# barronalex/Tacotron

Measured on AMD Instinct MI355X. Metric: mel-frames/sec (train step, batch=32 r=2), higher is better.
Workload: dtype f32

## Files before the change

include/taco_hip.h:

```cpp
#ifndef TACO_HIP_H
#define TACO_HIP_H

#include <stddef.h>
#include <stdint.h>

#ifdef __cplusplus
extern "C" {
#endif
#pragma GCC visibility push(default)

#define TACO_VERSION 120

#define TACO_OK 0
#define TACO_EINVAL (-1)
#define TACO_ELAUNCH (-2)
#define TACO_ENOTFOUND (-3)

#define TACO_ACT_NONE 0
#define TACO_ACT_RELU 1
#define TACO_ACT_SIGMOID 2
#define TACO_ACT_TANH 3

typedef struct TacoShape {
  int32_t B;
// ... 66 lines not shown
                                  int taps, int T, int pad_l, void* stream);
int taco_debug_bn_maxpool_fwd(const float* x, const float* gamma, const float* beta, float* y, int B, int T, int C, void* stream);
int taco_debug_bn_maxpool_bwd(const float* x, const float* gamma, const float* beta, const float* dy, float* dx, float* dgamma,
                              float* dbeta, int B, int T, int C, void* stream);
int taco_debug_bank_gather(const float* dbank, int lda, const float* const* WT, const float* residual, int ldr, float* dx_out, int ldc,
                           float* slabs, int64_t slab_floats, int M, int T, int F, int K, int N, int pad_l, int S, void* stream);
int taco_debug_conv_gemm_batch_atomic(const float* dbank, int lda, const float* const* WT, const float* residual, int ldr, float* dx_out,
                                      int ldc, int M, int T, int F, int K, int N, void* stream);
int taco_debug_conv_gemm_rowbias(const float* A, int lda, const float* W, int ldw, const float* rowb, int bias_stride, float* C, int ldc,
                                 int M, int T, int N, int K, void* stream);
int taco_debug_gemm_tn_group(int n, const float* const* A, const int* lda, const float* const* Y, const int* ldy, float* const* W,
                             const int* ldw, float* const* dbias, const int* M, const int* N, const int* K, const int* taps,
                             const int* T, const int* pad_l, void* stream);
int taco_debug_gemm_tn_strided(const float* A, int lda, int64_t strideA, const float* Y, int ldy, int64_t strideY, float* W, int ldw,
                               int64_t strideW, int M, int N, int K, int T, int pad_l, int batch, void* stream);

int taco_debug_embedding(const float* table, const int32_t* ids, float* out, int rows, int V, int width, void* stream);
int taco_debug_embedding_bwd(const float* dout, const int32_t* ids, float* dtable, int rows, int V, int width, void* stream);
int taco_debug_highway_combine(const float* th, const float* x, float* y, int M, void* stream);
int taco_debug_highway_combine_bwd(const float* th, const float* x, const float* dy, float* dth, float* dx, int M, void* stream);
int taco_debug_act_bwd(const float* y, const float* dy, const uint8_t* keep, float* dz, int64_t n, int act, void* stream);
int taco_debug_affine_act_bwd(const float* pre, const float* gamma, const float* dy, float* dz, float* dgamma, float* dbeta, int M,
                              int N, int act, void* stream);
int taco_debug_colsum_batched(const float* x, int ld, float* out, int B, int T, int N, void* stream);
int taco_debug_mask_rows(const float* x, const int32_t* len, float* y, int B, int T, int C, void* stream);
int taco_debug_center_rows(const float* x, const int32_t* len, float* out, int B, int T, int C, void* stream);
int taco_debug_mask_pos(float* g, int ldg, const float* y, int ldy, int rows, int cols, float scale, void* stream);
int taco_debug_zero_tail_rows(float* x0, int C0, float* x1, int C1, const int32_t* len, int B, int Td, void* stream);
int taco_debug_add(const float* a, const float* b, float* y, int64_t n, void* stream);
int taco_debug_l1_loss(const float* a0, const float* b0, float* grad0, int ldg0, int M0, int N0, const float* a1, const float* b1,
// ... 195 lines not shown
```

tacotron_amd/csrc/bf16x3.h:

```cpp
#pragma once
#include "common.h"

namespace {

typedef unsigned u32x4 __attribute__((ext_vector_type(4)));
typedef __bf16 bf16x8 __attribute__((ext_vector_type(8)));
struct Pl3 {
  u32x4 h, m, l;
};
__device__ __forceinline__ void split2(float x0, float x1, unsigned& h, unsigned& m, unsigned& l) {
  const unsigned u0 = __float_as_uint(x0), u1 = __float_as_uint(x1);
  h = __builtin_amdgcn_perm(u1, u0, 0x07060302u);
  const float r0 = x0 - __uint_as_float(u0 & 0xffff0000u), r1 = x1 - __uint_as_float(u1 & 0xffff0000u);
  const unsigned v0 = __float_as_uint(r0), v1 = __float_as_uint(r1);
  m = __builtin_amdgcn_perm(v1, v0, 0x07060302u);
  const float s0 = r0 - __uint_as_float(v0 & 0xffff0000u), s1 = r1 - __uint_as_float(v1 & 0xffff0000u);
  l = __builtin_amdgcn_perm(__float_as_uint(s1), __float_as_uint(s0), 0x07060302u);
}
__device__ __forceinline__ Pl3 split8(float f0, float f1, float f2, float f3, float f4, float f5, float f6, float f7) {
  unsigned h[4], m[4], l[4];
  split2(f0, f1, h[0], m[0], l[0]);
  split2(f2, f3, h[1], m[1], l[1]);
  split2(f4, f5, h[2], m[2], l[2]);
  split2(f6, f7, h[3], m[3], l[3]);
// ... 2 lines not shown
  p.m = u32x4{m[0], m[1], m[2], m[3]};
  p.l = u32x4{l[0], l[1], l[2], l[3]};
  return p;
}
__device__ __forceinline__ f32x16 mfma_bf(const u32x4& a, const u32x4& b, const f32x16& c) {
  return __builtin_amdgcn_mfma_f32_32x32x16_bf16(__builtin_bit_cast(bf16x8, a), __builtin_bit_cast(bf16x8, b), c, 0, 0, 0);
}
__device__ __forceinline__ void mfma6_2(f32x16& hi, f32x16& lo, const Pl3& a, const Pl3& b) {
  lo = mfma_bf(a.l, b.h, lo);
  hi = mfma_bf(a.h, b.h, hi);
  lo = mfma_bf(a.h, b.l, lo);
  lo = mfma_bf(a.m, b.m, lo);
  lo = mfma_bf(a.m, b.h, lo);
  lo = mfma_bf(a.h, b.m, lo);
}
__device__ __forceinline__ Pl3 zero_pl3() {
  Pl3 p;
  p.h = u32x4{0, 0, 0, 0}; p.m = p.h; p.l = p.h;
  return p;
}


inline bool env_bf16x() { return sw_on<SW_GEMM2_BF16X>(); }

inline int bf16x_max_chain() { return sw_int<SW_BF16X_MAX_CHAIN>(); }

}
```

tacotron_amd/csrc/gemm.hip:

```cpp
#include <algorithm>

#include "bf16x3.h"
#include "common.h"
#include "kernels.h"

namespace {

constexpr int BK = 16;

__device__ __forceinline__ float4 sel4(bool ok, const float4 t) {
  return make_float4(ok ? t.x : 0.f, ok ? t.y : 0.f, ok ? t.z : 0.f, ok ? t.w : 0.f);
}

struct RowInfo {
  int m;
  int t;
  bool ok;
};

template <int WM, int WN, bool VA, bool VB>
__global__ __launch_bounds__(256) void conv_gemm_kernel(ConvGemmBatch batch) {
  constexpr int BM = 64 * WM, BN = 64 * WN;
  constexpr int LDS_A = BM + 4, LDS_B = BN + 4;
  constexpr int A_PER = BM / 64;
// ... 881 lines not shown
  TACO_REQUIRE(bias_stride >= N, "%s: bias_stride must be >= N = %d, got %d", who, N, bias_stride);
  DoorOperands o;
  o.in(A, door_span(M, K, lda), "A");
  o.in(W, door_span(K, N, ldw), "W");
  o.in(rowb, door_span(M / T, N, bias_stride), "rowb");
  o.out(C, door_span(M, N, ldc), "C");
  TACO_TRY(o.check(who));
  ConvGemmProblem p;
  p.A = A; p.lda = lda; p.W = W; p.ldw = ldw; p.bias = rowb; p.C = C; p.ldc = ldc;
  p.M = M; p.N = N; p.K = K; p.taps = 1; p.pad_l = 0; p.act = TACO_ACT_NONE;
  p.T = T;
  p.bias_stride = bias_stride;
  return launch_conv_gemm(p, as_stream(stream));
}

extern "C" int taco_debug_gemm_tn_group(int n, const float* const* A, const int* lda, const float* const* Y, const int* ldy,
                                        float* const* W, const int* ldw, float* const* dbias, const int* M, const int* N, const int* K,
                                        const int* taps, const int* T, const int* pad_l, void* stream) {
  const char* who = "taco_debug_gemm_tn_group";
  TACO_REQUIRE(n >= 1 && n <= kMaxTnBatch, "%s: n must be in [1, %d], got %d", who, kMaxTnBatch, n);
  TACO_REQUIRE(A && lda && Y && ldy && W && ldw && M && N && K && taps && T && pad_l, "%s: a table is null", who);
  DoorOperands o;
  for (int i = 0; i < n; ++i) {
    TACO_REQUIRE(M[i] > 0 && M[i] <= kDoorMaxRows, "%s: M[%d] must be in [1, 2^22], got %d", who, i, M[i]);
    TACO_REQUIRE(T[i] > 0 && M[i] % T[i] == 0, "%s: T[%d] must be positive and divide M[%d] = %d, got %d", who, i, i, M[i], T[i]);
    TACO_REQUIRE(N[i] > 0 && N[i] <= kDoorMaxCols, "%s: N[%d] must be in [1, 2^14], got %d", who, i, N[i]);
    TACO_REQUIRE(K[i] > 0 && K[i] <= kDoorMaxCols, "%s: K[%d] must be in [1, 2^14], got %d", who, i, K[i]);
    TACO_REQUIRE(taps[i] >= 1 && taps[i] <= 64, "%s: taps[%d] must be in [1, 64], got %d", who, i, taps[i]);
    TACO_REQUIRE(pad_l[i] >= -64 && pad_l[i] <= 64, "%s: pad_l[%d] must be in [-64, 64], got %d", who, i, pad_l[i]);
    TACO_REQUIRE(lda[i] >= K[i], "%s: lda[%d] must be >= K = %d, got %d", who, i, K[i], lda[i]);
// ... 47 lines not shown
```

tacotron_amd/csrc/gemm2.hip:

```cpp
#include <algorithm>
#include <type_traits>

#include "bf16x3.h"
#include "common.h"
#include "kernels.h"

namespace {

__device__ __attribute__((aligned(16))) float g_zero4[4];

__device__ __forceinline__ void glds16(const float* g, float* lds_wave_base) {
  __builtin_amdgcn_global_load_lds((const __attribute__((address_space(1))) void*)g,
                                   (__attribute__((address_space(3))) void*)lds_wave_base, 16, 0, 0);
}
constexpr int kOOB = (int)0x80000000;
__device__ __forceinline__ __amdgpu_buffer_rsrc_t dma_rsrc(const float* base) {
  return __builtin_amdgcn_make_buffer_rsrc(const_cast<float*>(base), 0, 0x7fffffff, 0x00020000);
}
__device__ __forceinline__ void blds16(__amdgpu_buffer_rsrc_t rs, int voffset, int soffset, float* lds_wave_base) {
  __builtin_amdgcn_raw_ptr_buffer_load_lds(rs, (__attribute__((address_space(3))) void*)lds_wave_base, 16, voffset, soffset, 0, 0);
}
template <int N>
__device__ __forceinline__ void wait_vm() {
  asm volatile("s_waitcnt vmcnt(%0)" ::"n"(N) : "memory");
// ... 32 lines not shown
    f(std::integral_constant<int, I>{});
    static_for<I + 1, N>(f);
  }
}

constexpr int TM = 128, TN = 128;

struct Gemm2Args {
  ConvGemmBatch batch;
  int first[kMaxGemmBatch];
  int mt[kMaxGemmBatch];
  int xcd_map;
  int bk_pa[8], bk_a0[8], bk_na[8], bk_pb[8], bk_b0[8], bk_nb[8];
};

template <int BK, int NS, int BX = 0>
__global__ __launch_bounds__(256, 2) void conv_gemm2_kernel(Gemm2Args G) {
  static_assert(!BX || BK == 16, "the bf16x3 form works on 16-deep k-tiles (one v_mfma_f32_32x32x16_bf16 group per tile)");
  constexpr int SLOTS = BK / 4;
  constexpr int A_RPI = 64 / SLOTS;
  constexpr int A_INSTR = TM / A_RPI / 4;
  constexpr int B_INSTR = BX == 2 ? kWImgTileBytes / 4096 : BK / 2 / 4;
  constexpr int NLD = A_INSTR + B_INSTR;
  constexpr int A_FLOATS = TM * BK, B_FLOATS = BX == 2 ? kWImgTileBytes / 4 : BK * TN, STAGE = A_FLOATS + B_FLOATS;
  constexpr int SWZ_SH = BK == 32 ? 1 : 2;
  extern __shared__ __attribute__((aligned(16))) float smem[];

  int lin = blockIdx.x;
  int bank_pi = -1, bank_rel = 0;
  if (G.xcd_map == 2) {
    const int x = lin & 7, j = lin >> 3;
    if (j < G.bk_na[x]) { bank_pi = G.bk_pa[x]; bank_rel = G.bk_a0[x] + j; }
    else if (j < G.bk_na[x] + G.bk_nb[x]) { bank_pi = G.bk_pb[x]; bank_rel = G.bk_b0[x] + j - G.bk_na[x]; }
// ... 201 lines not shown
  auto compute_bi = [&](int stage, int fill_stage, auto fill_c) __attribute__((always_inline)) {
    constexpr bool fill = decltype(fill_c)::value;
    const uint32_t sb = lds0 + (uint32_t)stage * (STAGE * 4u);
    const uint32_t bb = sb + (uint32_t)(A_FLOATS * 4) + (uint32_t)lane * 16u;
    const f32x4 ra0 = dsr128<0>(sb + a_off[0]);
    const f32x4 ra1 = dsr128<0>(sb + a_off[NP - 1]);
    u32x4 pl[4][3];
    static_for<0, 4>([&](auto jc) {
      constexpr int j = decltype(jc)::value;
      static_for<0, 3>([&](auto pc) {
        constexpr int pp = decltype(pc)::value;
        pl[j][pp] = __builtin_bit_cast(u32x4, dsr128<(4 * pp + j) * 1024>(bb));
      });
    });
    __builtin_amdgcn_sched_barrier(0);
    acc_lo[2] = mfma_bf(pa_c.l, qb2_c.h, acc_lo[2]);
    acc_lo[3] = mfma_bf(pa_c.l, qb3_c.h, acc_lo[3]);
    acc[2] = mfma_bf(pa_c.h, qb2_c.h, acc[2]);
    acc[3] = mfma_bf(pa_c.h, qb3_c.h, acc[3]);
    acc_lo[2] = mfma_bf(pa_c.h, qb2_c.l, acc_lo[2]);
    acc_lo[3] = mfma_bf(pa_c.h, qb3_c.l, acc_lo[3]);
    if (fill) {
#pragma unroll
      for (int g = 0; g < NLD; ++g) issue_piece(g, fill_stage);
    }
    __builtin_amdgcn_sched_barrier(0);
    wait_lgkm<12>();
    __builtin_amdgcn_sched_barrier(0);
    acc_lo[2] = mfma_bf(pa_c.m, qb2_c.m, acc_lo[2]);
    acc_lo[3] = mfma_bf(pa_c.m, qb3_c.m, acc_lo[3]);
// ... 42 lines not shown
    __builtin_amdgcn_s_barrier();
    asm volatile("" ::: "memory");
    run_tile(it % NS, (it + NS - 1) % NS, std::true_type{});
    advance();
  }
  for (; it < nit; ++it) {
    wait_vm<0>();
    __builtin_amdgcn_s_barrier();
    asm volatile("" ::: "memory");
    run_tile(it % NS, 0, std::false_type{});
  }
  if constexpr (BX == 1) {
    MF6(2, pa_c, pb2_c);
    MF6(3, pa_c, pb3_c);
  }
  if constexpr (BX == 2) {
    MF6(2, pa_c, qb2_c);
    MF6(3, pa_c, qb3_c);
  }
  if constexpr (BX != 0) {
#pragma unroll
    for (int j = 0; j < 4; ++j) acc[j] += acc_lo[j];
  }
#undef MF6
  wait_vm<0>();

  const int n = n0 + 4 * li;
  if (P.pool == 2) {
    const bool col_ok = n + 3 < P.N;
    float sc[4] = {0.f, 0.f, 0.f, 0.f}, be[4] = {0.f, 0.f, 0.f, 0.f};
    if (col_ok) {
// ... 402 lines not shown
    }
  }
  if (do_bias && tid < 128 && n0 + tid < N) atomicAdd(P.dbias + n0 + tid, bsum);
}

inline bool al16(const void* p) { return (reinterpret_cast<uintptr_t>(p) & 15) == 0; }

struct Variant {
  int bk, ns;
};
Variant parse_variant(const char* e) {
  int bk = 0, ns = 0;
  if (e && sscanf(e, "%dx%d", &bk, &ns) == 2 && (bk == 16 || bk == 32) && ns >= 2 && ns <= 5) return Variant{bk, ns};
  return Variant{16, 4};
}
template <int BK, int NS, int BX = 0>
int launch_variant(const Gemm2Args& g, int tiles, hipStream_t s) {
  constexpr size_t smem = (size_t)NS * ((size_t)TM * BK * sizeof(float) + (BX == 2 ? (size_t)kWImgTileBytes : (size_t)BK * TN * sizeof(float)));
  static DynSmemOnce once;
  TACO_REQUIRE(ensure_dyn_smem(once, reinterpret_cast<const void*>(conv_gemm2_kernel<BK, NS, BX>), smem),
               "conv_gemm2: cannot reserve %zu bytes of LDS", smem);
  TACO_KLAUNCH((conv_gemm2_kernel<BK, NS, BX>), dim3(tiles), dim3(256), smem, s, g);
  return TACO_OK;
}


constexpr int kMaxWImgJobs = 40;
struct WImgJob {
  const float* W;
  unsigned short* img;
  int ldw, taps, K, N, kt, first;
};
struct WImgBatch {
  WImgJob j[kMaxWImgJobs];
  int n;
};
__global__ __launch_bounds__(256) void weight_image_kernel(WImgBatch B) {
// ... 215 lines not shown
  int64_t chain = 0;
  for (int i = 0; i < g.batch.n; ++i) {
    const ConvGemmProblem& p = g.batch.p[i];
    const int64_t c = p.it1 > 0 ? (int64_t)(p.it1 - p.it0) * 32 : (int64_t)p.taps * p.K;
    chain = c > chain ? c : chain;
  }
  if (env_bf16x() && chain <= bf16x_max_chain()) {
    bool img = sw_on<SW_GEMM2_BSPLIT>();
    for (int i = 0; i < g.batch.n && img; ++i) {
      ConvGemmProblem& p = g.batch.p[i];
      p.Wimg = weight_image_find(p.W, p.ldw, p.taps, p.K, p.Nld > 0 ? p.Nld : p.N, &p.img_its);
      img = p.Wimg != nullptr;
    }
    if (img) {
      __atomic_fetch_add(&g_img_launches, (int64_t)1, __ATOMIC_RELAXED);
      if (sw_int<SW_GEMM2_BI_NS>() == 4) return launch_variant<16, 4, 2>(g, tiles, stream);
      return launch_variant<16, 3, 2>(g, tiles, stream);
    }
    if (v.bk == 16 && v.ns == 3) return launch_variant<16, 3, 1>(g, tiles, stream);
    if (v.bk == 16 && v.ns == 5) return launch_variant<16, 5, 1>(g, tiles, stream);
    return launch_variant<16, 4, 1>(g, tiles, stream);
  }
  if (v.bk == 32 && v.ns == 2) return launch_variant<32, 2>(g, tiles, stream);
  if (v.bk == 32 && v.ns == 3) return launch_variant<32, 3>(g, tiles, stream);
  if (v.bk == 16 && v.ns == 3) return launch_variant<16, 3>(g, tiles, stream);
  if (v.bk == 16 && v.ns == 4) return launch_variant<16, 4>(g, tiles, stream);
  if (v.bk == 16 && v.ns == 5) return launch_variant<16, 5>(g, tiles, stream);
  return launch_variant<32, 2>(g, tiles, stream);
}

// ... 164 lines not shown
```

tacotron_amd/csrc/kernels.h:

```cpp
#pragma once
#include "common.h"
#include "stream.h"

constexpr int kMaxGemmBatch = 16;

struct ConvGemmProblem {
  const float* A = nullptr;
  const float* W = nullptr;
  const float* bias = nullptr;
  const float* scale = nullptr;
  const float* shift = nullptr;
  const float* residual = nullptr;
  const uint8_t* keep = nullptr;
  float* C = nullptr;
  float* Cpre = nullptr;
  int lda = 0, ldw = 0, ldr = 0, ldc = 0;
  int M = 0, N = 0, K = 0, taps = 1, T = 1, pad_l = 0, act = 0, flags = 0;
  int bias_stride = 0;
  int Nld = 0;
  int atomic_out = 0;
  float scale_mul = 1.f;
  int it0 = 0, it1 = 0;
  int bank_filters = 0;
  int pool = 0;
  const float* pool_x = nullptr;
  float* pool_dgamma = nullptr;
  float* pool_dbeta = nullptr;
  const void* Wimg = nullptr;
  int img_its = 0;
};
struct ConvGemmBatch {
  ConvGemmProblem p[kMaxGemmBatch];
  int n = 0;
};
struct GemmTnArgs {
  const float* A = nullptr;
  const float* Y = nullptr;
  float* W = nullptr;
  float* dbias = nullptr;
  int lda = 0, ldy = 0, ldw = 0;
  int M = 0, N = 0, K = 0, taps = 1, T = 1, pad_l = 0;
  int batch = 1;
  int64_t strideA = 0, strideY = 0, strideW = 0;
  int splits = 1, chunk = 0, flags = 0;
// ... 277 lines not shown
```

tacotron_amd/csrc/model.hip:

```cpp
#include <cstdarg>
#include <functional>
#include <map>
#include <mutex>
#include <tuple>
#include <vector>

#include "common.h"
#include "kernels.h"
#include "layout.h"

namespace {

struct Layouts {
  ParamLayout P;
  TransLayout T;
  WsLayout Wtrain, Winfer;
};

const Layouts& layouts_for(const TacoShape& s) {
  static std::mutex mu;
  static std::map<std::tuple<int, int, int, int, int, int>, Layouts*> cache;
  std::lock_guard<std::mutex> g(mu);
  auto key = std::make_tuple(s.B, s.Tt, s.Td, s.r, s.V, s.S > 1 ? s.S : 1);
  auto it = cache.find(key);
// ... 557 lines not shown
  const float* wx = ws + W.dc_wx;
  job(P + PL.mem_w, kAtt, ws + W.bc_wmx, 2 * kCb, 2 * kCb, kAtt);
  job(wx + (int64_t)(kPre2 + R80) * kDec, kDec, ws + W.bc_wxct, kAtt, kAtt, kDec);
  job(wx + (int64_t)kPre2 * kDec, kDec, fa, NO, R80, kDec);
  job(P + PL.out_proj.w, R80, wot, kDec, kDec, R80);
  job(ws + W.dc_wo, dec_out_cols(r), wot + (int64_t)R80 * kDec, kDec, kDec, kAtt);
  job(ws + W.dc_wp1o, kPre1, wot + (int64_t)(R80 + kAtt) * kDec, kDec, kDec, kPre1);
  TACO_TRY(launch_transpose_batch(tb, s));
  return launch_conv_gemm(dense_problem(fa, NO, wot, kDec, nullptr, ws + W.bc_wdx, kDec, kDec, kDec, R80, TACO_ACT_NONE), s);
}

struct BwdScratch {
  float *gA, *gB, *gC, *gD, *gE, *gF, *gG;
  float *alt_dpj1 = nullptr, *alt_dz1 = nullptr, *alt_dpool = nullptr;
  bool dx_zeroed = false;
};

int cbhg_bwd(const float* P, const float* PT, float* G, const CbhgP& c, const CbhgT& t, const float* x, const float* dOut,
             int B, int T, const CbhgBufs& w, const BwdScratch& sc, float* dx_out, int seg_after_p1, int seg_after_bank, hipStream_t s) {
  const int M = B * T, KC = c.K * kCb;
  float* dxg = sc.gC;
  float* rh = sc.gD;
  BiGruBwdWeights bw;
  for (int d = 0; d < 2; ++d) {
    bw.wghT[d] = PT + t.wghT[d];
    bw.wchT[d] = PT + t.wchT[d];
  }
  TACO_TRY(launch_bigru_bwd(dOut, w.out, w.ruc, bw, c.spk ? w.h0 : nullptr, dxg, rh, c.spk ? w.dh0 : nullptr, B, T, s));
  const GruP* g[2] = {&c.fw, &c.bw};
  TnGroup gru_group(s);
  for (int d = 0; d < 2; ++d) {
    const float* dG = dxg + d * 3 * kCb;
    const float* dC = dG + 2 * kCb;
    TACO_TRY(tn(w.h[4], kCb, kCb, dG, 6 * kCb, 2 * kCb, G + g[d]->wg, 2 * kCb, M, T, 0, s, 1, G + g[d]->bg));
    TACO_TRY(tn(w.out + d * kCb, 2 * kCb, kCb, dG, 6 * kCb, 2 * kCb, G + g[d]->wg + (int64_t)kCb * 2 * kCb, 2 * kCb, M, T,
                d == 0 ? 1 : -1, s));
    TACO_TRY(tn(w.h[4], kCb, kCb, dC, 6 * kCb, kCb, G + g[d]->wc, kCb, M, T, 0, s, 1, G + g[d]->bc));
    TACO_TRY(tn(rh + d * kCb, 2 * kCb, kCb, dC, 6 * kCb, kCb, G + g[d]->wc + (int64_t)kCb * kCb, kCb, M, T, 0, s));
    if (c.spk) {
      const float* dG0 = dG + (int64_t)(d == 0 ? 0 : T - 1) * 6 * kCb;
      TACO_TRY(tn(w.h0, kCb, kCb, dG0, T * 6 * kCb, 2 * kCb, G + g[d]->wg + (int64_t)kCb * 2 * kCb, 2 * kCb, B, B, 0, s));
    }
  }
// ... 333 lines not shown
  const Layouts& L = layouts_for(*shape);
  const ParamLayout& PL = L.P;
  const TransLayout& TL = L.T;
  const WsLayout& W = L.Wtrain;
  float* ws = static_cast<float*>(workspace);
  float* G = grads;
  const float* P = params;
  const int B = shape->B, Tt = shape->Tt, Td = shape->Td, r = shape->r, R80 = kMel * r;
  const int M1 = B * Tt, MD = B * Td, M2 = MD * r, F = Td * r;
  float* PT = ws + W.paramsT;

  TACO_TRY(register_weight_images(L, W, P, ws, true, 0, false));
  TACO_TRY(register_weight_images(L, W, P, ws, true, 1, false));
  const bool side_tn_on = !sw_on<SW_NO_SIDE_TN>();
  const bool own_dx = side_tn_on && side_stream_or_null() != nullptr;
  {
    InitBatch ib;
    TACO_TRY(ib.fill(G, PL.total));
    TACO_TRY(ib.fill(ws + W.dkeys, (int64_t)M1 * 2 * kAtt));
    TACO_TRY(ib.fill(ws + W.bc_g, W.bc_cp + kPre1 - W.bc_g));
    TACO_TRY(ib.fill(ws + W.xchg, decoder_xchg_bytes(B, Tt) / 4));
    if (own_dx) {
      if (!taco_deterministic()) TACO_TRY(ib.copy(ws + W.post_dx, ws + W.ds2s, (int64_t)M2 * kMel));
      else TACO_TRY(ib.fill(ws + W.post_dx, (int64_t)M2 * kMel));
      if (!PL.enc.spk || spk_fused_form(PL.enc)) TACO_TRY(ib.fill(ws + W.enc_dx, (int64_t)M1 * kCb));
    }
    TACO_TRY(launch_init_batch(ib, s));
  }
  BwdScratch sc{ws + W.gA, ws + W.gB, ws + W.gC, ws + W.gD, ws + W.gE, ws + W.gF, ws + W.gG};
  CbhgBufs pb = cbhg_bufs(ws, W.post), eb = cbhg_bufs(ws, W.enc);

  const float* dOutPad = ws + W.dout_pad;
  float* dPostOut = sc.gG;
  TACO_TRY(launch_conv_gemm(dense_problem(dOutPad, 1028, PT + TL.post_dense, 2 * kCb, nullptr, dPostOut, 2 * kCb, M2, 2 * kCb,
                                          1028 , TACO_ACT_NONE), s));
  hipStream_t side = side_fork(s);
  TACO_TRY(tn(pb.out, 2 * kCb, 2 * kCb, dOutPad, 1028, kFft, G + PL.post_dense.w, kFft, M2, M2, 0, side, 1, G + PL.post_dense.b, 1028));
  BwdScratch scp = sc;
  float* dPostIn = sc.gC;
  const bool side_tn = side != s && side_tn_on;
  if (side_tn) {
    scp.alt_dpj1 = ws + W.post_dpj1; scp.alt_dz1 = ws + W.post_dz1; scp.alt_dpool = ws + W.post_dpool;
    dPostIn = ws + W.post_dx;
    scp.dx_zeroed = own_dx;
  }
  pb.tapsplit = ws + W.tapsplit;
  pb.tapsplit_floats = W.tapsplit_floats;
  {
    ScopedRoute route(side_tn ? side : nullptr);
    TACO_TRY(cbhg_bwd(P, PT, G, PL.post, TL.post, seq2seq_output, dPostOut, B, F, pb, scp, dPostIn, -1, -1, s));
  }
  float* dS2S = ws + W.ds2s_tot;
  if (side_tn && own_dx && !taco_deterministic()) dS2S = dPostIn;
  else TACO_TRY(launch_add(ws + W.ds2s, dPostIn, dS2S, (int64_t)MD * R80, s));
  TACO_TRY(side_join(s, side));

  float* gs = ws + W.gstash;
  const float* st = ws + W.stash;
  {
    DecBwdArgs a;
    DecWeights& w = a.wT;
    w.pre_w1 = PT + TL.dec_pre1; w.pre_w2 = PT + TL.dec_pre2; w.in_w = PT + TL.in_proj;
// ... 260 lines not shown
```

tacotron_amd/csrc/stream.h:

```cpp
#pragma once
#include "common.h"

hipEvent_t taco_tail_take(hipStream_t s, hipEvent_t* start);

#define TACO_KLAUNCH(kernel, grid, block, smem, stream, ...)                                                        \
  do {                                                                                                              \
    hipEvent_t tst__ = nullptr;                                                                                     \
    hipEvent_t tev__ = taco_tail_take(stream, &tst__);                                                              \
    if (tev__) hipExtLaunchKernelGGL(kernel, grid, block, smem, stream, tst__, tev__, 0, __VA_ARGS__);              \
    else hipLaunchKernelGGL(kernel, grid, block, smem, stream, __VA_ARGS__);                                        \
  } while (0)

int taco_memset_async(void* p, int v, size_t bytes, hipStream_t s, const char* what);
int taco_upload_async(void* dst, const void* host_src, size_t bytes, hipStream_t s, const char* what);

struct StreamMark {
  hipEvent_t ev = nullptr;
  bool tail = false;
  hipStream_t producer = nullptr;
  hipEvent_t* fallback = nullptr;
};
StreamMark stream_mark(hipStream_t producer, hipStream_t waiter, hipEvent_t* fallback);
int stream_wait_mark(hipStream_t waiter, StreamMark m);
int stream_wait(hipStream_t waiter, hipStream_t producer, hipEvent_t* fallback);

hipStream_t side_stream_or_null();
hipStream_t side_fork(hipStream_t s);
int side_join(hipStream_t s, hipStream_t side);
StreamMark side_mark_images(hipStream_t side, hipStream_t s);

constexpr int kGradSegments = 5;
int record_segment(int seg, hipStream_t on);
int wait_grad_segment(int seg, hipStream_t stream);

int tn_route(hipStream_t s, hipStream_t* out);
void tn_queue_reset();

struct ScopedRoute {
  const hipStream_t prev;
  explicit ScopedRoute(hipStream_t side);
  ScopedRoute(const ScopedRoute&) = delete;
  ~ScopedRoute();
};

// ... 11 lines not shown
```

tacotron_amd/csrc/stream.hip:

```cpp
#include "stream.h"
#include "kernels.h"

#include <stdarg.h>

namespace {
constexpr int kTailRing = 64, kTailStreams = 8, kPlanWords = 8, kPlans = 32;
hipStream_t const kDepMany = reinterpret_cast<hipStream_t>(~(uintptr_t)0);
struct TailTrack {
  bool used = false;
  hipStream_t s = nullptr;
  hipEvent_t ring[kTailRing] = {};
  int next = 0;
  int tail_slot = -1;
  hipEvent_t tail = nullptr;
  bool has_dep = false;
  hipStream_t dep = nullptr;
  int launches = 0;
  int tail_idx = -1;
  bool declined = false;
  int dev = 0;
  uint64_t stamp = 0;
  bool armed = false;
  hipEvent_t arm_start = nullptr, arm_stop = nullptr;
  int arm_launches = 0;
// ... 305 lines not shown
  int pos = 0;
  for (int i = 0; i < r.n; ++i) {
    const int w = snprintf(buf + pos, cap - pos, "%s\n", r.label[i]);
    if (w < 0 || pos + w >= cap) break;
    pos += w;
  }
  buf[pos < cap ? pos : cap - 1] = 0;
  return r.n;
}

namespace {
struct SideStream {
  hipStream_t side = nullptr;
  hipEvent_t ev_fork = nullptr, ev_join = nullptr;
  hipEvent_t ev_img = nullptr;
  bool off = false;
  hipEvent_t ev_seg[kGradSegments] = {nullptr, nullptr, nullptr, nullptr, nullptr};
  hipEvent_t ev_seg_use[kGradSegments] = {nullptr, nullptr, nullptr, nullptr, nullptr};
  bool seg_recorded = false;
};
SideStream& side_stream() {
  static thread_local SideStream ss[16];
  int dev = 0;
  (void)hipGetDevice(&dev);
  SideStream& x = ss[dev & 15];
  if (!x.side && !x.off) {
    if (sw_on<SW_NO_OVERLAP>() || hipStreamCreateWithFlags(&x.side, hipStreamNonBlocking) != hipSuccess ||
        hipEventCreateWithFlags(&x.ev_fork, hipEventDisableTiming) != hipSuccess ||
        hipEventCreateWithFlags(&x.ev_join, hipEventDisableTiming) != hipSuccess) {
      x.side = nullptr;
// ... 9 lines not shown
  SideStream& x = side_stream();
  if (x.off || (g_prof_mask & 16)) return s;
  return stream_wait(x.side, s, &x.ev_fork) == TACO_OK ? x.side : s;
}
int side_join(hipStream_t s, hipStream_t side) {
  if (side == s) return TACO_OK;
  if (stream_wait(s, side, &side_stream().ev_join) != TACO_OK) {
    taco_set_error("side_join: event record/wait failed");
    return TACO_ELAUNCH;
  }
  return TACO_OK;
}
StreamMark side_mark_images(hipStream_t side, hipStream_t s) {
  return stream_mark(side, s, &side_stream().ev_img);
}
int record_segment(int seg, hipStream_t on) {
  SideStream& x = side_stream();
  if (!x.ev_seg[seg] && hipEventCreateWithFlags(&x.ev_seg[seg], hipEventDisableTiming) != hipSuccess) {
    taco_set_error("taco_backward: cannot create the gradient-segment event");
    return TACO_ELAUNCH;
  }
  bool owned = false;
  if (hipEvent_t t = tail_steal(on, x.ev_seg[seg], &owned)) {
    if (owned) x.ev_seg[seg] = t;
    x.ev_seg_use[seg] = t;
  } else {
    hipStream_t at = on;
    if (x.side && x.side != on && !x.off && stream_wait(x.side, on, nullptr) == TACO_OK) at = x.side;
    if (hipEventRecord(x.ev_seg[seg], at) != hipSuccess) {
      taco_set_error("taco_backward: hipEventRecord(segment %d) failed", seg);
// ... 57 lines not shown
```

tacotron_amd/lib.py:

```python
from __future__ import annotations

import collections
import ctypes as C
import math
import os

from . import QUEUES_SET_BY_USER as _QUEUES_SET_BY_USER, TORCH_IMPORTED_FIRST as _TORCH_IMPORTED_FIRST

import numpy as np
import torch

from .argcheck import (float_arg, int_arg, no_overlap, on_gpu, pow2_bins, step_q_arg, tensor_arg,
                       host_int32 as _host_int32, own_or_given as _own_or_given, unit_interval as _unit_interval)

HW_QUEUES_LATE = (not _QUEUES_SET_BY_USER) and (_TORCH_IMPORTED_FIRST or (torch.cuda.is_available() and torch.cuda.is_initialized()))


def effective_hw_queues() -> int:
    if HW_QUEUES_LATE:
        return 4
    try:
        return int(os.environ.get('GPU_MAX_HW_QUEUES', '4'))
    except ValueError:
        return 4
# ... 57 lines not shown
    'taco_debug_gemm_naive': (C.c_int, [_P, _I, _P, _I, _P, _P, _I, _I, _I, _I, _I, _I, _I, _I, _P]),
    'taco_bigru_fwd': (C.c_int, [_P] * 12 + [_I, _I, _P]),
    'taco_debug_bigru_rec_fwd': (C.c_int, [_P] * 8 + [_I, _I, _P]),
    'taco_debug_bigru_bwd': (C.c_int, [_P] * 11 + [_I, _I, _P]),
    'taco_debug_highway_stack_fwd': (C.c_int, [_P] * 10 + [_I, _I, _I, _P]),
    'taco_debug_highway_stack_bwd': (C.c_int, [_P] * 8 + [_I, _I, _P]),
    'taco_debug_prenet_fwd': (C.c_int, [_P] * 9 + [_I, _P]),
    'taco_debug_prenet_bwd': (C.c_int, [_P] * 10 + [_I, _P]),
    'taco_debug_conv_bank_pool_fwd': (C.c_int, [_P, _I, _P, _P, _P, _P, C.c_float, _P, _P, _I, _I, _I, _I, _I, _I, _P]),
    'taco_debug_conv_gemm_pool_bwd': (C.c_int, [_P, _I, _P, _I, _P, _P, _P, C.c_float, _P, _I, _P, _P, _I, _I, _I, _I, _I, _I, _P]),
    'taco_debug_bn_maxpool_fwd': (C.c_int, [_P] * 4 + [_I, _I, _I, _P]),
    'taco_debug_bn_maxpool_bwd': (C.c_int, [_P] * 7 + [_I, _I, _I, _P]),
    'taco_debug_bank_gather': (C.c_int, [_P, _I, _P, _P, _I, _P, _I, _P, C.c_int64, _I, _I, _I, _I, _I, _I, _I, _P]),
    'taco_debug_conv_gemm_batch_atomic': (C.c_int, [_P, _I, _P, _P, _I, _P, _I, _I, _I, _I, _I, _I, _P]),
    'taco_debug_conv_gemm_rowbias': (C.c_int, [_P, _I, _P, _I, _P, _I, _P, _I, _I, _I, _I, _I, _P]),
    'taco_debug_gemm_tn_group': (C.c_int, [_I] + [_P] * 13 + [_P]),
    'taco_debug_gemm_tn_strided': (C.c_int, [_P, _I, C.c_int64, _P, _I, C.c_int64, _P, _I, C.c_int64, _I, _I, _I, _I, _I, _I, _P]),
    'taco_debug_embedding': (C.c_int, [_P, _P, _P, _I, _I, _I, _P]),
    'taco_debug_embedding_bwd': (C.c_int, [_P, _P, _P, _I, _I, _I, _P]),
    'taco_debug_highway_combine': (C.c_int, [_P, _P, _P, _I, _P]),
    'taco_debug_highway_combine_bwd': (C.c_int, [_P] * 5 + [_I, _P]),
    'taco_debug_act_bwd': (C.c_int, [_P, _P, _P, _P, C.c_int64, _I, _P]),
    'taco_debug_affine_act_bwd': (C.c_int, [_P] * 6 + [_I, _I, _I, _P]),
    'taco_debug_colsum_batched': (C.c_int, [_P, _I, _P, _I, _I, _I, _P]),
    'taco_debug_mask_rows': (C.c_int, [_P, _P, _P, _I, _I, _I, _P]),
    'taco_debug_center_rows': (C.c_int, [_P, _P, _P, _I, _I, _I, _P]),
    'taco_debug_mask_pos': (C.c_int, [_P, _I, _P, _I, _I, _I, C.c_float, _P]),
    'taco_debug_zero_tail_rows': (C.c_int, [_P, _I, _P, _I, _P, _I, _I, _P]),
    'taco_debug_add': (C.c_int, [_P, _P, _P, C.c_int64, _P]),
    'taco_debug_l1_loss': (C.c_int, [_P, _P, _P, _I, _I, _I, _P, _P, _P, _I, _I, _I, _P, _P, _P, _P]),
# ... 56 lines not shown
    'taco_audio_features_workspace_bytes': (C.c_int64, [_I, _I]),
    'taco_audio_features': (C.c_int, [_P, C.POINTER(C.c_int32), _P, _P, _P, _P, _P, _P, _I, _I, _I, _I, _I, _P]),
    'taco_wave_resample': (C.c_int, [_P, C.c_int64, _I, _I, _P, _P, _I, _I, _I, _I, _P, _I, _I, _P]),
    'taco_fill_bernoulli': (C.c_int, [_P, C.c_int64, C.c_float, C.c_uint64, _P]),
    'taco_tensor_stats_plan_bytes': (C.c_int64, [C.POINTER(C.c_int64), _I]),
    'taco_tensor_stats_plan': (C.c_int, [C.POINTER(C.c_int64), _I, C.c_int64, _P, C.c_int64, C.POINTER(C.c_int32)]),
    'taco_tensor_stats_workspace_bytes': (C.c_int64, [_I, _I, _I]),
    'taco_tensor_stats': (C.c_int, [_P, _P, _P, _I, _I, _I, _I, _I, _P, _P, _P, _P, _P]),
    'taco_profile_enable': (C.c_int, [_I]),
    'taco_debug_last_cluster': (C.c_int, [_I]),
    'taco_profile_read': (C.c_int, [_I, C.POINTER(C.c_float), _I]),
    'taco_debug_profile_labels': (C.c_int, [_I, C.c_char_p, _I]),
    'taco_profile_read2': (C.c_int, [_I, C.POINTER(C.c_float), C.POINTER(C.c_double), _I]),
}
for _name, (_res, _args) in EXPORTS.items():
    _fn = getattr(_lib, _name)
    _fn.restype = _res
    _fn.argtypes = _args


def last_error() -> str:
    return _lib.taco_last_error_string().decode()


def _check(rc: int, what: str):
    if rc != 0:
        raise TacoError('%s failed (rc=%d): %s' % (what, rc, last_error()))


def ptr(t):
# ... 412 lines not shown
    ins += [('residual', residual, _span(M, N, ldr), True)]
    _flat_args(who, ins, [('dx_out', dx_out, _span(M, N, ldc), False)])
    _check(_lib.taco_debug_conv_gemm_batch_atomic(ptr(dbank), lda, _ptr_table(WT), ptr(residual), ldr, ptr(dx_out), ldc, M, T, F, K, N,
                                                  stream_ptr()), 'taco_debug_conv_gemm_batch_atomic')


def debug_conv_gemm_rowbias(A, W, rowb, C_out, M, T, N, K, bias_stride=None, lda=None, ldw=None, ldc=None):
    who = 'debug_conv_gemm_rowbias'
    M, T, N, K = _gemm_dims(who, M, T, N=N, K=K)
    lda, ldw, ldc = _pitch(who, 'lda', lda, K), _pitch(who, 'ldw', ldw, N), _pitch(who, 'ldc', ldc, N)
    bias_stride = _pitch(who, 'bias_stride', bias_stride, N)
    _flat_args(who, [('A', A, _span(M, K, lda), False), ('W', W, _span(K, N, ldw), False), ('rowb', rowb, _span(M // T, N, bias_stride), False)],
               [('C_out', C_out, _span(M, N, ldc), False)])
    _check(_lib.taco_debug_conv_gemm_rowbias(ptr(A), lda, ptr(W), ldw, ptr(rowb), bias_stride, ptr(C_out), ldc, M, T, N, K, stream_ptr()),
           'taco_debug_conv_gemm_rowbias')


def debug_gemm_tn_group(problems):
    who = 'debug_gemm_tn_group'
    if not isinstance(problems, (list, tuple)) or not 1 <= len(problems) <= 26:
        raise ValueError('%s: problems must be a list of 1 to 26 dicts' % who)
    ins, outs, rows = [], [], []
    for i, p in enumerate(problems):
        w = '%s: problems[%d]' % (who, i)
        M, T, N, K = _gemm_dims(w, p['M'], p['T'], N=p['N'], K=p['K'])
        taps, pad_l = int_arg(w, 'taps', p['taps'], 1, 64), int_arg(w, 'pad_l', p['pad_l'], -64, 64)
        lda, ldy, ldw = _pitch(w, 'lda', p.get('lda'), K), _pitch(w, 'ldy', p.get('ldy'), N), _pitch(w, 'ldw', p.get('ldw'), N)
        ins += [('A[%d]' % i, p['A'], _span(M, K, lda), False), ('Y[%d]' % i, p['Y'], _span(M, N, ldy), False)]
        outs += [('W[%d]' % i, p['W'], _span(taps * K, N, ldw), False), ('dbias[%d]' % i, p.get('dbias'), N, True)]
        rows.append((lda, ldy, ldw, M, N, K, taps, T, pad_l))
# ... 1421 lines not shown
```

Measured before the change: 1.643 million.

## Use one-plane bf16 A operand in post-dense dx GEMM and overlap gradient init on side stream

```diff
diff --git a/include/taco_hip.h b/include/taco_hip.h
--- a/include/taco_hip.h
+++ b/include/taco_hip.h
@@ -104,6 +104,8 @@
                              const int* T, const int* pad_l, void* stream);
 int taco_debug_gemm_tn_strided(const float* A, int lda, int64_t strideA, const float* Y, int ldy, int64_t strideY, float* W, int ldw,
                                int64_t strideW, int M, int N, int K, int T, int pad_l, int batch, void* stream);
+int taco_debug_conv_gemm_planes(const float* A, int lda, const float* W, int ldw, const float* bias, float* C, int ldc, int M, int N,
+                                int K, int taps, int T, int pad_l, int act, int a_planes, void* stream);
 
 int taco_debug_embedding(const float* table, const int32_t* ids, float* out, int rows, int V, int width, void* stream);
 int taco_debug_embedding_bwd(const float* dout, const int32_t* ids, float* dtable, int rows, int V, int width, void* stream);
diff --git a/tacotron_amd/csrc/bf16x3.h b/tacotron_amd/csrc/bf16x3.h
--- a/tacotron_amd/csrc/bf16x3.h
+++ b/tacotron_amd/csrc/bf16x3.h
@@ -40,6 +40,17 @@
   lo = mfma_bf(a.m, b.h, lo);
   lo = mfma_bf(a.h, b.m, lo);
 }
+__device__ __forceinline__ u32x4 hi8(float f0, float f1, float f2, float f3, float f4, float f5, float f6, float f7) {
+  return u32x4{__builtin_amdgcn_perm(__float_as_uint(f1), __float_as_uint(f0), 0x07060302u),
+               __builtin_amdgcn_perm(__float_as_uint(f3), __float_as_uint(f2), 0x07060302u),
+               __builtin_amdgcn_perm(__float_as_uint(f5), __float_as_uint(f4), 0x07060302u),
+               __builtin_amdgcn_perm(__float_as_uint(f7), __float_as_uint(f6), 0x07060302u)};
+}
+__device__ __forceinline__ void mfma3_2(f32x16& hi, f32x16& lo, const u32x4& ah, const Pl3& b) {
+  hi = mfma_bf(ah, b.h, hi);
+  lo = mfma_bf(ah, b.l, lo);
+  lo = mfma_bf(ah, b.m, lo);
+}
 __device__ __forceinline__ Pl3 zero_pl3() {
   Pl3 p;
   p.h = u32x4{0, 0, 0, 0}; p.m = p.h; p.l = p.h;
diff --git a/tacotron_amd/csrc/gemm.hip b/tacotron_amd/csrc/gemm.hip
--- a/tacotron_amd/csrc/gemm.hip
+++ b/tacotron_amd/csrc/gemm.hip
@@ -919,6 +919,33 @@
   return launch_conv_gemm(p, as_stream(stream));
 }
 
+extern "C" int taco_debug_conv_gemm_planes(const float* A, int lda, const float* W, int ldw, const float* bias, float* C, int ldc, int M,
+                                           int N, int K, int taps, int T, int pad_l, int act, int a_planes, void* stream) {
+  const char* who = "taco_debug_conv_gemm_planes";
+  TACO_REQUIRE(M > 0 && M <= kDoorMaxRows, "%s: M must be in [1, 2^22], got %d", who, M);
+  TACO_REQUIRE(T > 0 && M % T == 0, "%s: T must be positive and divide M = %d, got %d", who, M, T);
+  TACO_REQUIRE(N > 0 && N <= kDoorMaxCols, "%s: N must be in [1, 2^14], got %d", who, N);
+  TACO_REQUIRE(K > 0 && K <= kDoorMaxCols, "%s: K must be in [1, 2^14], got %d", who, K);
+  TACO_REQUIRE(taps >= 1 && taps <= 64, "%s: taps must be in [1, 64], got %d", who, taps);
+  TACO_REQUIRE(pad_l >= -64 && pad_l <= 64, "%s: pad_l must be in [-64, 64], got %d", who, pad_l);
+  TACO_REQUIRE(act >= TACO_ACT_NONE && act <= TACO_ACT_TANH, "%s: act must be in [0, %d], got %d", who, TACO_ACT_TANH, act);
+  TACO_REQUIRE(a_planes == 0 || a_planes == 1, "%s: a_planes must be 0 or 1, got %d", who, a_planes);
+  TACO_REQUIRE(lda >= K, "%s: lda must be >= K = %d, got %d", who, K, lda);
+  TACO_REQUIRE(ldw >= N, "%s: ldw must be >= N = %d, got %d", who, N, ldw);
+  TACO_REQUIRE(ldc >= N, "%s: ldc must be >= N = %d, got %d", who, N, ldc);
+  DoorOperands o;
+  o.in(A, door_span(M, K, lda), "A");
+  o.in(W, door_span((int64_t)taps * K, N, ldw), "W");
+  o.in_opt(bias, (size_t)N * sizeof(float), "bias");
+  o.out(C, door_span(M, N, ldc), "C");
+  TACO_TRY(o.check(who));
+  ConvGemmProblem p;
+  p.A = A; p.lda = lda; p.W = W; p.ldw = ldw; p.bias = bias; p.C = C; p.ldc = ldc;
+  p.M = M; p.N = N; p.K = K; p.taps = taps; p.T = T; p.pad_l = pad_l; p.act = act;
+  p.a_planes = a_planes;
+  return launch_conv_gemm(p, as_stream(stream));
+}
+
 extern "C" int taco_debug_gemm_tn_group(int n, const float* const* A, const int* lda, const float* const* Y, const int* ldy,
                                         float* const* W, const int* ldw, float* const* dbias, const int* M, const int* N, const int* K,
                                         const int* taps, const int* T, const int* pad_l, void* stream) {
diff --git a/tacotron_amd/csrc/gemm2.hip b/tacotron_amd/csrc/gemm2.hip
--- a/tacotron_amd/csrc/gemm2.hip
+++ b/tacotron_amd/csrc/gemm2.hip
@@ -70,9 +70,10 @@
   int bk_pa[8], bk_a0[8], bk_na[8], bk_pb[8], bk_b0[8], bk_nb[8];
 };
 
-template <int BK, int NS, int BX = 0>
+template <int BK, int NS, int BX = 0, bool A1 = false>
 __global__ __launch_bounds__(256, 2) void conv_gemm2_kernel(Gemm2Args G) {
   static_assert(!BX || BK == 16, "the bf16x3 form works on 16-deep k-tiles (one v_mfma_f32_32x32x16_bf16 group per tile)");
+  static_assert(!A1 || BX == 2, "the one-plane A operand exists in the B-image form only");
   constexpr int SLOTS = BK / 4;
   constexpr int A_RPI = 64 / SLOTS;
   constexpr int A_INSTR = TM / A_RPI / 4;
@@ -304,6 +305,37 @@
       });
     });
     __builtin_amdgcn_sched_barrier(0);
+    if constexpr (A1) {
+      acc[2] = mfma_bf(pa_c.h, qb2_c.h, acc[2]);
+      acc[3] = mfma_bf(pa_c.h, qb3_c.h, acc[3]);
+      acc_lo[2] = mfma_bf(pa_c.h, qb2_c.l, acc_lo[2]);
+      acc_lo[3] = mfma_bf(pa_c.h, qb3_c.l, acc_lo[3]);
+      if (fill) {
+#pragma unroll
+        for (int g = 0; g < NLD; ++g) issue_piece(g, fill_stage);
+      }
+      __builtin_amdgcn_sched_barrier(0);
+      wait_lgkm<12>();
+      __builtin_amdgcn_sched_barrier(0);
+      acc_lo[2] = mfma_bf(pa_c.h, qb2_c.m, acc_lo[2]);
+      acc_lo[3] = mfma_bf(pa_c.h, qb3_c.m, acc_lo[3]);
+      const u32x4 ah_n = hi8(ra0[0], ra0[1], ra0[2], ra0[3], ra1[0], ra1[1], ra1[2], ra1[3]);
+      __builtin_amdgcn_sched_barrier(0);
+      wait_lgkm<0>();
+      __builtin_amdgcn_sched_barrier(0);
+      pa_c.h = ah_n;
+      acc[0] = mfma_bf(pa_c.h, pl[0][0], acc[0]);
+      acc[1] = mfma_bf(pa_c.h, pl[1][0], acc[1]);
+      acc_lo[0] = mfma_bf(pa_c.h, pl[0][2], acc_lo[0]);
+      acc_lo[1] = mfma_bf(pa_c.h, pl[1][2], acc_lo[1]);
+      acc_lo[0] = mfma_bf(pa_c.h, pl[0][1], acc_lo[0]);
+      acc_lo[1] = mfma_bf(pa_c.h, pl[1][1], acc_lo[1]);
+      qb2_c.h = pl[2][0]; qb2_c.m = pl[2][1]; qb2_c.l = pl[2][2];
+      qb3_c.h = pl[3][0]; qb3_c.m = pl[3][1]; qb3_c.l = pl[3][2];
+      asm volatile("" : "+v"(qb2_c.h), "+v"(qb2_c.m), "+v"(qb2_c.l), "+v"(qb3_c.h), "+v"(qb3_c.m), "+v"(qb3_c.l));
+      __builtin_amdgcn_sched_barrier(0);
+      return;
+    }
     acc_lo[2] = mfma_bf(pa_c.l, qb2_c.h, acc_lo[2]);
     acc_lo[3] = mfma_bf(pa_c.l, qb3_c.h, acc_lo[3]);
     acc[2] = mfma_bf(pa_c.h, qb2_c.h, acc[2]);
@@ -376,7 +408,11 @@
     MF6(2, pa_c, pb2_c);
     MF6(3, pa_c, pb3_c);
   }
-  if constexpr (BX == 2) {
+  if constexpr (BX == 2 && A1) {
+    mfma3_2(acc[2], acc_lo[2], pa_c.h, qb2_c);
+    mfma3_2(acc[3], acc_lo[3], pa_c.h, qb3_c);
+  }
+  if constexpr (BX == 2 && !A1) {
     MF6(2, pa_c, qb2_c);
     MF6(3, pa_c, qb3_c);
   }
@@ -809,13 +845,13 @@
   if (e && sscanf(e, "%dx%d", &bk, &ns) == 2 && (bk == 16 || bk == 32) && ns >= 2 && ns <= 5) return Variant{bk, ns};
   return Variant{16, 4};
 }
-template <int BK, int NS, int BX = 0>
+template <int BK, int NS, int BX = 0, bool A1 = false>
 int launch_variant(const Gemm2Args& g, int tiles, hipStream_t s) {
   constexpr size_t smem = (size_t)NS * ((size_t)TM * BK * sizeof(float) + (BX == 2 ? (size_t)kWImgTileBytes : (size_t)BK * TN * sizeof(float)));
   static DynSmemOnce once;
-  TACO_REQUIRE(ensure_dyn_smem(once, reinterpret_cast<const void*>(conv_gemm2_kernel<BK, NS, BX>), smem),
+  TACO_REQUIRE(ensure_dyn_smem(once, reinterpret_cast<const void*>(conv_gemm2_kernel<BK, NS, BX, A1>), smem),
                "conv_gemm2: cannot reserve %zu bytes of LDS", smem);
-  TACO_KLAUNCH((conv_gemm2_kernel<BK, NS, BX>), dim3(tiles), dim3(256), smem, s, g);
+  TACO_KLAUNCH((conv_gemm2_kernel<BK, NS, BX, A1>), dim3(tiles), dim3(256), smem, s, g);
   return TACO_OK;
 }
 
@@ -1061,6 +1097,12 @@
     }
     if (img) {
       __atomic_fetch_add(&g_img_launches, (int64_t)1, __ATOMIC_RELAXED);
+      bool a1 = true;
+      for (int i = 0; i < g.batch.n; ++i) a1 = a1 && g.batch.p[i].a_planes == 1;
+      if (a1) {
+        if (sw_int<SW_GEMM2_BI_NS>() == 4) return launch_variant<16, 4, 2, true>(g, tiles, stream);
+        return launch_variant<16, 3, 2, true>(g, tiles, stream);
+      }
       if (sw_int<SW_GEMM2_BI_NS>() == 4) return launch_variant<16, 4, 2>(g, tiles, stream);
       return launch_variant<16, 3, 2>(g, tiles, stream);
     }
diff --git a/tacotron_amd/csrc/kernels.h b/tacotron_amd/csrc/kernels.h
--- a/tacotron_amd/csrc/kernels.h
+++ b/tacotron_amd/csrc/kernels.h
@@ -28,6 +28,7 @@
   float* pool_dbeta = nullptr;
   const void* Wimg = nullptr;
   int img_its = 0;
+  int a_planes = 0;
 };
 struct ConvGemmBatch {
   ConvGemmProblem p[kMaxGemmBatch];
diff --git a/tacotron_amd/csrc/model.hip b/tacotron_amd/csrc/model.hip
--- a/tacotron_amd/csrc/model.hip
+++ b/tacotron_amd/csrc/model.hip
@@ -595,6 +595,8 @@
   float *gA, *gB, *gC, *gD, *gE, *gF, *gG;
   float *alt_dpj1 = nullptr, *alt_dz1 = nullptr, *alt_dpool = nullptr;
   bool dx_zeroed = false;
+  const StreamMark* init_done = nullptr;
+  hipStream_t init_stream = nullptr;
 };
 
 int cbhg_bwd(const float* P, const float* PT, float* G, const CbhgP& c, const CbhgT& t, const float* x, const float* dOut,
@@ -608,6 +610,7 @@
     bw.wchT[d] = PT + t.wchT[d];
   }
   TACO_TRY(launch_bigru_bwd(dOut, w.out, w.ruc, bw, c.spk ? w.h0 : nullptr, dxg, rh, c.spk ? w.dh0 : nullptr, B, T, s));
+  if (sc.init_done && stream_wait_mark(s, *sc.init_done) != TACO_OK) TACO_TRY(side_join(s, sc.init_stream));
   const GruP* g[2] = {&c.fw, &c.bw};
   TnGroup gru_group(s);
   for (int d = 0; d < 2; ++d) {
@@ -971,7 +974,8 @@
   TACO_TRY(register_weight_images(L, W, P, ws, true, 1, false));
   const bool side_tn_on = !sw_on<SW_NO_SIDE_TN>();
   const bool own_dx = side_tn_on && side_stream_or_null() != nullptr;
-  {
+  const bool init_beside = side_stream_or_null() != nullptr && !taco_deterministic();
+  auto init_accumulators = [&](hipStream_t q) -> int {
     InitBatch ib;
     TACO_TRY(ib.fill(G, PL.total));
     TACO_TRY(ib.fill(ws + W.dkeys, (int64_t)M1 * 2 * kAtt));
@@ -982,16 +986,26 @@
       else TACO_TRY(ib.fill(ws + W.post_dx, (int64_t)M2 * kMel));
       if (!PL.enc.spk || spk_fused_form(PL.enc)) TACO_TRY(ib.fill(ws + W.enc_dx, (int64_t)M1 * kCb));
     }
-    TACO_TRY(launch_init_batch(ib, s));
-  }
+    return launch_init_batch(ib, q);
+  };
+  if (!init_beside) TACO_TRY(init_accumulators(s));
   BwdScratch sc{ws + W.gA, ws + W.gB, ws + W.gC, ws + W.gD, ws + W.gE, ws + W.gF, ws + W.gG};
   CbhgBufs pb = cbhg_bufs(ws, W.post), eb = cbhg_bufs(ws, W.enc);
 
   const float* dOutPad = ws + W.dout_pad;
   float* dPostOut = sc.gG;
-  TACO_TRY(launch_conv_gemm(dense_problem(dOutPad, 1028, PT + TL.post_dense, 2 * kCb, nullptr, dPostOut, 2 * kCb, M2, 2 * kCb,
-                                          1028 , TACO_ACT_NONE), s));
+  {
+    ConvGemmProblem dx = dense_problem(dOutPad, 1028, PT + TL.post_dense, 2 * kCb, nullptr, dPostOut, 2 * kCb, M2, 2 * kCb,
+                                       1028 , TACO_ACT_NONE);
+    dx.a_planes = 1;
+    TACO_TRY(launch_conv_gemm(dx, s));
+  }
   hipStream_t side = side_fork(s);
+  StreamMark init_mark;
+  if (init_beside) {
+    TACO_TRY(init_accumulators(side));
+    if (side != s) init_mark = side_mark_init(side, s);
+  }
   TACO_TRY(tn(pb.out, 2 * kCb, 2 * kCb, dOutPad, 1028, kFft, G + PL.post_dense.w, kFft, M2, M2, 0, side, 1, G + PL.post_dense.b, 1028));
   BwdScratch scp = sc;
   float* dPostIn = sc.gC;
@@ -1003,6 +1017,10 @@
   }
   pb.tapsplit = ws + W.tapsplit;
   pb.tapsplit_floats = W.tapsplit_floats;
+  if (init_beside && side != s) {
+    scp.init_done = &init_mark;
+    scp.init_stream = side;
+  }
   {
     ScopedRoute route(side_tn ? side : nullptr);
     TACO_TRY(cbhg_bwd(P, PT, G, PL.post, TL.post, seq2seq_output, dPostOut, B, F, pb, scp, dPostIn, -1, -1, s));
diff --git a/tacotron_amd/csrc/stream.h b/tacotron_amd/csrc/stream.h
--- a/tacotron_amd/csrc/stream.h
+++ b/tacotron_amd/csrc/stream.h
@@ -28,6 +28,7 @@
 hipStream_t side_fork(hipStream_t s);
 int side_join(hipStream_t s, hipStream_t side);
 StreamMark side_mark_images(hipStream_t side, hipStream_t s);
+StreamMark side_mark_init(hipStream_t side, hipStream_t s);
 
 constexpr int kGradSegments = 5;
 int record_segment(int seg, hipStream_t on);
diff --git a/tacotron_amd/csrc/stream.hip b/tacotron_amd/csrc/stream.hip
--- a/tacotron_amd/csrc/stream.hip
+++ b/tacotron_amd/csrc/stream.hip
@@ -343,6 +343,7 @@
   hipStream_t side = nullptr;
   hipEvent_t ev_fork = nullptr, ev_join = nullptr;
   hipEvent_t ev_img = nullptr;
+  hipEvent_t ev_init = nullptr;
   bool off = false;
   hipEvent_t ev_seg[kGradSegments] = {nullptr, nullptr, nullptr, nullptr, nullptr};
   hipEvent_t ev_seg_use[kGradSegments] = {nullptr, nullptr, nullptr, nullptr, nullptr};
@@ -382,6 +383,9 @@
 StreamMark side_mark_images(hipStream_t side, hipStream_t s) {
   return stream_mark(side, s, &side_stream().ev_img);
 }
+StreamMark side_mark_init(hipStream_t side, hipStream_t s) {
+  return stream_mark(side, s, &side_stream().ev_init);
+}
 int record_segment(int seg, hipStream_t on) {
   SideStream& x = side_stream();
   if (!x.ev_seg[seg] && hipEventCreateWithFlags(&x.ev_seg[seg], hipEventDisableTiming) != hipSuccess) {
diff --git a/tacotron_amd/lib.py b/tacotron_amd/lib.py
--- a/tacotron_amd/lib.py
+++ b/tacotron_amd/lib.py
@@ -95,6 +95,7 @@
     'taco_debug_bank_gather': (C.c_int, [_P, _I, _P, _P, _I, _P, _I, _P, C.c_int64, _I, _I, _I, _I, _I, _I, _I, _P]),
     'taco_debug_conv_gemm_batch_atomic': (C.c_int, [_P, _I, _P, _P, _I, _P, _I, _I, _I, _I, _I, _I, _P]),
     'taco_debug_conv_gemm_rowbias': (C.c_int, [_P, _I, _P, _I, _P, _I, _P, _I, _I, _I, _I, _I, _P]),
+    'taco_debug_conv_gemm_planes': (C.c_int, [_P, _I, _P, _I, _P, _P, _I, _I, _I, _I, _I, _I, _I, _I, _I, _P]),
     'taco_debug_gemm_tn_group': (C.c_int, [_I] + [_P] * 13 + [_P]),
     'taco_debug_gemm_tn_strided': (C.c_int, [_P, _I, C.c_int64, _P, _I, C.c_int64, _P, _I, C.c_int64, _I, _I, _I, _I, _I, _I, _P]),
     'taco_debug_embedding': (C.c_int, [_P, _P, _P, _I, _I, _I, _P]),
@@ -181,6 +182,8 @@
     'taco_profile_read2': (C.c_int, [_I, C.POINTER(C.c_float), C.POINTER(C.c_double), _I]),
 }
 for _name, (_res, _args) in EXPORTS.items():
+    if _name == 'taco_debug_conv_gemm_planes' and os.environ.get('TACO_LIB') and not hasattr(_lib, _name):
+        continue
     _fn = getattr(_lib, _name)
     _fn.restype = _res
     _fn.argtypes = _args
@@ -623,6 +626,20 @@
                [('C_out', C_out, _span(M, N, ldc), False)])
     _check(_lib.taco_debug_conv_gemm_rowbias(ptr(A), lda, ptr(W), ldw, ptr(rowb), bias_stride, ptr(C_out), ldc, M, T, N, K, stream_ptr()),
            'taco_debug_conv_gemm_rowbias')
+
+
+def debug_conv_gemm_planes(A, W, C_out, M, N, K, taps=1, T=None, pad_l=0, act=0, bias=None, a_planes=0, lda=None, ldw=None, ldc=None):
+    who = 'debug_conv_gemm_planes'
+    M, T, N, K = _gemm_dims(who, M, M if T is None else T, N=N, K=K)
+    taps = int_arg(who, 'taps', taps, 1, 64)
+    pad_l = int_arg(who, 'pad_l', pad_l, -64, 64)
+    act = int_arg(who, 'act', act, 0, 3)
+    a_planes = int_arg(who, 'a_planes', a_planes, 0, 1)
+    lda, ldw, ldc = _pitch(who, 'lda', lda, K), _pitch(who, 'ldw', ldw, N), _pitch(who, 'ldc', ldc, N)
+    _flat_args(who, [('A', A, _span(M, K, lda), False), ('W', W, _span(taps * K, N, ldw), False), ('bias', bias, N, True)],
+               [('C_out', C_out, _span(M, N, ldc), False)])
+    _check(_lib.taco_debug_conv_gemm_planes(ptr(A), lda, ptr(W), ldw, ptr(bias), ptr(C_out), ldc, M, N, K, taps, T, pad_l, act, a_planes,
+                                            stream_ptr()), 'taco_debug_conv_gemm_planes')
 
 
 def debug_gemm_tn_group(problems):
```

Result: no change. 1.641 million (-0.1%).
